# ShadenSmith/splatt

Measured on AMD Instinct MI355X. Metric: mttkrp_gflops, higher is better.
Workload: dtype f64; 1 GPU; model=amazon-shaped CPD-ALS, nnz=1741809018, cp_rank=16, csf=all, tiling=none, parallelism=medium-grid [1, 1, 1] x1 (RCCL/xGMI)

## Files before the change

### csrc/hip/launchers.hpp

```cpp
#pragma once
#include <cstdint>

namespace splatt_store {
struct bf16 { uint16_t v; };
}

namespace splatt {
namespace hip {

using splatt_store::bf16;

int kernels_arch();
const char * error_string(int rc);

template <typename V>
int mttkrp_csf3(int which, const int64_t * fptr0, const int32_t * fids0,
                const int64_t * fptr1, const int32_t * fids1,
                const int32_t * fids2, const V * vals, int64_t nslices,
                int64_t nfibs, int64_t nnz, const V * Ma, const V * Mb,
                V * out, int rank, void * stream);

template <typename V, typename S = V, typename VS = V>
int mttkrp_flat(const int32_t * key, const int64_t * rowptr, int64_t nrows,
                int64_t p0, const int32_t * const * idx,
                const S * const * mats, const VS * vals, int64_t nnz, V * out,
                int rank, int nother, void * stream);

template <typename V>
int mttkrp_flat5(const int32_t * key, const int32_t * const * idx,
                 const V * const * mats, const V * vals,
                 const int64_t * blk_start, const int64_t * blk_end,
                 const int32_t * blk_row0, int64_t nblocks, int32_t chunk,
                 int32_t dim0, V * out, int rank, int nother, void * stream);
template <typename V, typename S = V>
int mttkrp_flat6(const int32_t * pack, const S * const * mats,
                 const V * vals, const int64_t * blk_start,
                 const int64_t * blk_end, const int32_t * blk_row0,
                 int64_t nblocks, int32_t chunk, int32_t dim0, V * out,
                 int rank, int nother, void * stream);

template <typename VS>
int mttkrp_strip(const int32_t * key, const int32_t * const * idx,
                 const double * const * mats, const VS * vals,
                 const int32_t * s_row0, const int32_t * s_nrows,
                 const int32_t * s_flags, const int64_t * s_bounds,
                 int ngroups, int64_t nstrips, int tile_rows, int wgs,
                 int64_t nnz, double * out, int rank, int nother,
                 void * stream, uint32_t * pace, int pace_us);
int strip_wgs(int rank, int nother, bool vals32, int tile_rows);
int strip_wall_khz();

template <typename V>
int mttkrp_det6(const int32_t * pack, const V * const * mats, const V * vals,
                const int64_t * blk_start, const int64_t * blk_end,
                const int32_t * blk_row0, const int64_t * blk_bucket_p0,
                int64_t nblocks, int32_t chunk, int32_t dim0,
                int64_t nrows_out, int64_t nbuckets, V * outb, V * side,
                V * out, int rank, int nother, void * stream);
int64_t flat_det_ws(int64_t nnz, int rank);
template <typename V>
int mttkrp_flat_det(const int32_t * key, const int32_t * const * idx,
                    const V * const * mats, const V * vals, int64_t nnz,
                    V * out, V * side, int64_t side_elems, int rank,
                    int nother, void * stream);

template <typename V>
int gram(const V * A, int64_t n, int F, V * G, void * stream);
template <typename V>
int gram_det(const V * A, int64_t n, int F, V * Gpart, int64_t nparts, V * G,
             void * stream);
template <typename V>
int rowsolve(const V * A, const V * B, V * C, int64_t n, int F,
             void * stream);
template <typename V>
int spd_inverse(const V * G, V * Ginv, int F, void * stream);
int colacc(const double * A, int64_t n, int F, int which, double * out,
           void * stream);
int colscale(double * A, int64_t n, int F, const double * lam, void * stream);
int coldot(const double * X, const double * A, int64_t n, int F, double * out,
           void * stream);
int als_prep(const double * const * grams, int ngrams, double reg,
             double * Ginv, int F, double * zero_gram, double * lam_init,
             double * zero_inner, void * stream);

int als_tail(const double * K, const double * Ginv, int64_t n, int F,
             double * A, double * lam, double * gram, double * inner,
             void * stream);
int64_t als_tail_cap_rows();

int64_t complete_slot_elems(int F);
int complete_segments(const int32_t * const * idx,
                      const double * const * mats, int nother,
                      const double * vals, const int64_t * seg_start,
                      const int32_t * seg_len, const int32_t * seg_row,
                      const int32_t * seg_slot, int64_t seg0, int64_t nseg,
                      int64_t slot0, int F, double reg, double * ws,
                      double * out, void * stream);
int complete_reduce(const double * ws, const int32_t * mrow,
                    const int64_t * mslot, int64_t m0, int64_t nm,
                    int64_t slot0, int F, double reg, double * out,
                    void * stream);
// ... 35 lines not shown
```

### csrc/hip/mttkrp_strip.hip

```cpp
#include <hip/hip_runtime.h>
#include <cstdint>

#include <type_traits>

#include "device_common.hpp"
#include "launchers.hpp"

namespace {

constexpr int STRIP_THREADS = 1024;
constexpr int STRIP_PAD = 2;

template <typename T, int N>
__device__ __forceinline__ void ldnt_vec(const T * p, T (&r)[N]) {
  if constexpr (N == 1) {
    r[0] = ldnt(p);
  } else {
    using VT = T __attribute__((ext_vector_type(N)));
    const VT v = __builtin_nontemporal_load(reinterpret_cast<const VT *>(p));
    #pragma unroll
    for (int i = 0; i < N; ++i) r[i] = v[i];
  }
}

struct StripArgs {
  const int32_t * key, * i0, * i1, * i2;
  const double * m0, * m1, * m2;
  const int32_t * row0, * nrows, * flags;
  const int64_t * bounds;
  int ngroups;
  int64_t nnz;
  uint32_t * pace;
  int64_t budget;
};

constexpr int PACE_ARRIVALS = 0;
constexpr int PACE_TIMEOUTS = 32;
constexpr int PACE_LONGEST = 64;
constexpr int PACE_WORDS = 96;

template <int F, int NOTHER, typename VS>
__global__ void __launch_bounds__(STRIP_THREADS)
mttkrp_strip_kern(const StripArgs a, const VS * __restrict__ vals,
                  int64_t nstrips, int tile_rows,
                  double * __restrict__ out) {
  constexpr int R = WAVE / F;
  constexpr int W = 32;
  constexpr int EPL = (F >= W) ? 1 : W / F;
  constexpr int VPL = (sizeof(VS) == 8 && EPL > 1) ? EPL / 2 : EPL;
  constexpr int NVL = EPL / VPL;
  constexpr int CH = W / NVL;
  constexpr int GB = 8;
  constexpr int LD = F + STRIP_PAD;
  extern __shared__ double tile[];

  const int32_t * __restrict__ key = a.key;
  const int32_t * __restrict__ i0 = a.i0;
  const int32_t * __restrict__ i1 = a.i1;
  const int32_t * __restrict__ i2 = a.i2;
  const double * __restrict__ m0 = a.m0;
  const double * __restrict__ m1 = a.m1;
  const double * __restrict__ m2 = a.m2;

  uint32_t ticket = 0;
  bool waiting = true;
  int64_t longest = 0;
  auto pace = [&]() {
    if (!a.pace) return;
    __syncthreads();
    if (threadIdx.x == 0) {
      uint32_t * arrivals = a.pace + PACE_ARRIVALS;
      __hip_atomic_fetch_add(arrivals, 1u, __ATOMIC_RELAXED,
                             __HIP_MEMORY_SCOPE_AGENT);
      const uint32_t target = ++ticket * gridDim.x;
      if (waiting) {
        const int64_t t0 = (int64_t)wall_clock64();
        while (__hip_atomic_load(arrivals, __ATOMIC_RELAXED,
                                 __HIP_MEMORY_SCOPE_AGENT) < target) {
          if ((int64_t)wall_clock64() - t0 >= a.budget) {
            atomicAdd(a.pace + PACE_TIMEOUTS, 1u);
            waiting = false;
            break;
          }
          __builtin_amdgcn_s_sleep(8);
        }
        const int64_t dt = (int64_t)wall_clock64() - t0;
        if (dt > longest) longest = dt;
      }
    }
    __syncthreads();
  };

  const int lane = threadIdx.x & (WAVE - 1);
  const int c = lane % F;
  const int g = lane / F;
  const int gbase = g * F;
  const int slot = c & (W / EPL - 1);
  const int nlg = (blockDim.x / WAVE) * R;
  const int gid = (threadIdx.x / WAVE) * R + g;

  for (int64_t s = blockIdx.x; s - blockIdx.x < nstrips; s += gridDim.x) {
    if (s >= nstrips) {
      for (int grp = 0; grp < a.ngroups; ++grp) pace();
      break;
    }
    const int32_t row0 = a.row0[s];
    const int nr = a.nrows[s] < tile_rows ? a.nrows[s] : tile_rows;
    const int fl = a.flags[s];
    const int64_t * bnd = a.bounds + s * (a.ngroups + 1);

    for (int e = threadIdx.x; e < nr * LD; e += blockDim.x) tile[e] = 0.0;
    __syncthreads();

    int32_t cur = -1;
    double acc = 0.0;
    auto flush = [&]() {
      const uint32_t lr = (uint32_t)(cur - row0);
      if (lr < (uint32_t)nr) unsafeAtomicAdd(&tile[lr * LD + c], acc);
    };
    auto fold = [&](int32_t k, double x) {
      if (k != cur) {
        flush();
        acc = 0.0;
        cur = k;
      }
      acc += x;
    };
    auto scalar = [&](int64_t pa, int64_t pb) {
      for (int64_t p = pa; p < pb; ++p) {
        double x = (double)ldnt(&vals[p]) * m0[(int64_t)ldnt(&i0[p]) * F + c]
                   * ldnt(&m1[(int64_t)ldnt(&i1[p]) * F + c]);
        if constexpr (NOTHER > 2)
          x *= ldnt(&m2[(int64_t)ldnt(&i2[p]) * F + c]);
        fold(ldnt(&key[p]), x);
      }
    };

    for (int grp = 0; grp < a.ngroups; ++grp) {
      const int64_t p0 = bnd[grp], p1 = bnd[grp + 1];
      const int64_t wlo = p0 / W;
// ... 14 lines not shown
        #pragma unroll
        for (int k = 0; k < NVL; ++k)
          ldnt_vec(vals + pw + k * CH + slot * VPL, vreg[k]);
        #pragma unroll
        for (int k = 0; k < NVL; ++k) {
          #pragma unroll 1
          for (int h = 0; h < CH; h += GB) {
            const int ub = k * CH + h;
            double vv[GB], a0[GB], a1[GB], a2[GB];
            #pragma unroll
            for (int u = 0; u < GB; ++u) {
              const int src = gbase + ub / EPL + u / EPL;
              vv[u] = (double)__shfl(vreg[k][u % VPL],
                                     gbase + h / VPL + u / VPL, WAVE);
              const int32_t j0 = __shfl(i0reg[u % EPL], src, WAVE);
              const int32_t j1 = __shfl(i1reg[u % EPL], src, WAVE);
              a0[u] = m0[(int64_t)j0 * F + c];
              a1[u] = ldnt(&m1[(int64_t)j1 * F + c]);
              if constexpr (NOTHER > 2) {
                const int32_t j2 = __shfl(i2reg[u % EPL], src, WAVE);
                a2[u] = ldnt(&m2[(int64_t)j2 * F + c]);
              }
            }
            #pragma unroll
            for (int u = 0; u < GB; ++u) {
              double x = vv[u] * a0[u] * a1[u];
              if constexpr (NOTHER > 2) x *= a2[u];
              const int32_t k = __shfl(kreg[u % EPL],
                                       gbase + ub / EPL + u / EPL, WAVE);
              if (ub + u >= lo && ub + u < hi) fold(k, x);
            }
          }
        }
      }

      if (wend > whi && gid == nlg - 1)
        scalar(whi * W > p0 ? whi * W : p0, p1);
      if (grp + 1 < a.ngroups) pace();
    }
    flush();
    __syncthreads();

    for (int e = threadIdx.x; e < nr * F; e += blockDim.x) {
      const int lr = e / F, cc = e % F;
      const double v = tile[lr * LD + cc];
      double * o = &out[(int64_t)(row0 + lr) * F + cc];
      if ((lr == 0 && (fl & 1)) || (lr == nr - 1 && (fl & 2)))
        atomic_add_g(o, v);
      else
        *o = v;
    }
    if (a.pace) pace(); else __syncthreads();
  }
  if (a.pace && threadIdx.x == 0 && longest > 0)
    atomicMax(a.pace + PACE_LONGEST,
              (uint32_t)(longest < 0xFFFFFFFFll ? longest : 0xFFFFFFFFll));
}

inline int lds_limit() {
  static int limit = -1;
  if (limit < 0) {
    int dev = 0, v = 0;
    if (hipGetDevice(&dev) != hipSuccess
        || hipDeviceGetAttribute(&v, hipDeviceAttributeMaxSharedMemoryPerBlock,
                                 dev) != hipSuccess)
      return 0;
    limit = v;
  }
  return limit;
}

inline int cu_count() {
  static int n = -1;
  if (n < 0) {
    int dev = 0, v = 0;
    if (hipGetDevice(&dev) != hipSuccess
        || hipDeviceGetAttribute(&v, hipDeviceAttributeMultiprocessorCount,
                                 dev) != hipSuccess)
      return 0;
    n = v;
  }
  return n;
}

inline int wall_khz() {
  static int khz = -1;
  if (khz < 0) {
    int dev = 0, v = 0;
    if (hipGetDevice(&dev) != hipSuccess
        || hipDeviceGetAttribute(&v, hipDeviceAttributeWallClockRate, dev)
               != hipSuccess || v <= 0)
      return 0;
    khz = v;
  }
  return khz;
}

struct StripLaunch {
  StripArgs a;
  const void * vals;
  int64_t nstrips;
  int wgs;
  int tile_rows;
  double * out;
  hipStream_t st;
};

template <int F, int NOTHER, typename VS>
int strip_inst(const StripLaunch * L, int lds, int * wgs) {
  static int lds_set = 0;
  auto kern = mttkrp_strip_kern<F, NOTHER, VS>;
  if (lds > lds_set) {
    const hipError_t e = hipFuncSetAttribute(
        reinterpret_cast<const void *>(kern),
        hipFuncAttributeMaxDynamicSharedMemorySize, lds);
    if (e != hipSuccess) return (int)e;
    lds_set = lds;
  }
  if (!L) {
    int per_cu = 0;
    const hipError_t e = hipOccupancyMaxActiveBlocksPerMultiprocessor(
        &per_cu, kern, STRIP_THREADS, (size_t)lds);
    if (e != hipSuccess) return (int)e;
    *wgs = per_cu * cu_count();
    return wall_khz() > 0 ? 0 : (int)hipErrorInvalidDevice;
  }
  if (L->a.pace) {
    const hipError_t e = hipMemsetAsync(
        L->a.pace, 0, PACE_WORDS * sizeof(uint32_t), L->st);
    if (e != hipSuccess) return (int)e;
  }
  const int64_t n = L->nstrips < L->wgs ? L->nstrips : L->wgs;
  hipLaunchKernelGGL(kern, dim3((uint32_t)n), dim3(STRIP_THREADS),
                     (size_t)lds, L->st, L->a,
                     static_cast<const VS *>(L->vals), L->nstrips,
                     L->tile_rows, L->out);
  return launch_rc();
}

template <typename VS>
int strip_dispatch(const StripLaunch * L, int tile_rows, int rank, int nother,
                   int * wgs) {
  if (!(rank == 16 || rank == 32 || rank == 64) || nother < 2 || nother > 3
      || tile_rows < 1)
    return -1;
  const int64_t lds = (int64_t)tile_rows * (rank + STRIP_PAD) * 8;
  if (lds > lds_limit()) return -2;
#define SI(F_, N_) return strip_inst<F_, N_, VS>(L, (int)lds, wgs)
#define SF(N_) \
  switch (rank) { case 16: SI(16, N_); case 32: SI(32, N_); \
                  default: SI(64, N_); }
  if (nother == 2) { SF(2); }
  SF(3);
#undef SF
#undef SI
}

}

namespace splatt {
namespace hip {

int strip_wgs(int rank, int nother, bool vals32, int tile_rows) {
  int wgs = 0;
  const int rc = vals32
      ? strip_dispatch<float>(nullptr, tile_rows, rank, nother, &wgs)
      : strip_dispatch<double>(nullptr, tile_rows, rank, nother, &wgs);
  return rc == 0 ? wgs : 0;
}

template <typename VS>
int mttkrp_strip(const int32_t * key, const int32_t * const * idx,
                 const double * const * mats, const VS * vals,
                 const int32_t * s_row0, const int32_t * s_nrows,
                 const int32_t * s_flags, const int64_t * s_bounds,
                 int ngroups, int64_t nstrips, int tile_rows, int wgs,
                 int64_t nnz, double * out, int rank, int nother,
                 void * stream, uint32_t * pace, int pace_us) {
  if (nstrips <= 0) return 0;
  if (wgs < 1 || ngroups < 1 || nother < 2 || nother > 3 || pace_us < 0)
    return -1;
  uintptr_t bits = (uintptr_t)key | (uintptr_t)vals;
  for (int t = 0; t < nother; ++t) bits |= (uintptr_t)idx[t];
  if (bits & 127) return -1;
  StripLaunch L{{key, idx[0], idx[1], nother > 2 ? idx[2] : nullptr, mats[0],
                 mats[1], nother > 2 ? mats[2] : nullptr, s_row0, s_nrows,
                 s_flags, s_bounds, ngroups, nnz, pace,
                 (int64_t)pace_us * wall_khz() / 1000},
                vals, nstrips, wgs, tile_rows, out, (hipStream_t)stream};
  return strip_dispatch<VS>(&L, tile_rows, rank, nother, nullptr);
}

#define STRIP_SIG(VS)                                                      \
  const int32_t *, const int32_t * const *, const double * const *,        \
  const VS *, const int32_t *, const int32_t *, const int32_t *,           \
  const int64_t *, int, int64_t, int, int, int64_t, double *, int, int,    \
  void *, uint32_t *, int
template int mttkrp_strip<double>(STRIP_SIG(double));
template int mttkrp_strip<float>(STRIP_SIG(float));
#undef STRIP_SIG

int strip_wall_khz() { return wall_khz(); }

}
}
```

### csrc/pybind.cpp

```cpp
#include <torch/extension.h>
#include <array>
#include <string>
#include <vector>

#include "core/types.hpp"
#include "core/sptensor.hpp"
#include "core/csf.hpp"
#include "core/mttkrp_cpu.hpp"
#include "core/matrix.hpp"
#include "core/cpd.hpp"
#include "core/io.hpp"
#include "core/partition.hpp"
#include "hip/launchers.hpp"

namespace sp = splatt;
namespace gpu = splatt::hip;
using torch::Tensor;


template <typename T> struct Tag { using type = T; };
#define TAG_TYPE(tag) typename decltype(tag)::type

template <typename T>
static constexpr torch::ScalarType dtype_of() {
// ... 454 lines not shown
    rp = rowptr_ptr(*rowptr, out);
  }
  return gpu::mttkrp_flat<V, S, VS>(kp, rp, rp ? rowptr->numel() - 1 : 0, p0,
                                    ip.data(), mp.data(), vp, nnz, op, rank,
                                    (int)nother, (void *)stream);
}

static void py_gpu_mttkrp_flat(Tensor key, std::vector<Tensor> idx,
                               std::vector<Tensor> mats, Tensor vals,
                               Tensor out, int64_t stream) {
  TORCH_CHECK(!mats.empty(), "flat kernel supports 3..8 modes");
  by_store(vals, mats[0], [&](auto v, auto s) {
    using V = TAG_TYPE(v);
    using S = TAG_TYPE(s);
    const int rc = flat_launch<V, S, V>(c10::nullopt, 0, key, idx, mats, vals,
                                        out, stream);
    check_rc(rc, "flat MTTKRP",
             std::string(std::is_same<S, float>::value ? "f32" : "bf16")
             + " factor store needs rank in {4,8,16,32,64}");
  });
}

static bool py_gpu_mttkrp_flat_rp(Tensor rowptr, int64_t p0,
                                  std::vector<Tensor> idx,
                                  std::vector<Tensor> mats, Tensor vals,
                                  Tensor out, int64_t stream) {
  TORCH_CHECK(!mats.empty(), "flat kernel supports 3..8 modes");
  return by_store(vals, mats[0], [&](auto v, auto s) {
    using V = TAG_TYPE(v);
    const int rc = flat_launch<V, TAG_TYPE(s), V>(rowptr, p0, c10::nullopt,
                                                  idx, mats, vals, out,
                                                  stream);
    if (rc > 0) check_rc(rc, "flat MTTKRP");
    return rc == 0;
  });
}

static bool py_gpu_mttkrp_flat_v32(c10::optional<Tensor> rowptr, int64_t p0,
                                   c10::optional<Tensor> key,
                                   std::vector<Tensor> idx,
                                   std::vector<Tensor> mats, Tensor vals32,
                                   Tensor out, int64_t stream) {
  const int rc = flat_launch<double, double, float>(rowptr, p0, key, idx, mats,
                                                    vals32, out, stream);
  if (rc > 0) check_rc(rc, "flat MTTKRP");
  return rc == 0;
}

static bool py_mttkrp_strip_gpu(Tensor key, std::vector<Tensor> idx,
                                std::vector<Tensor> mats, Tensor vals,
                                Tensor s_row0, Tensor s_nrows, Tensor s_flags,
                                Tensor s_bounds, int64_t tile_rows,
                                int64_t wgs, Tensor out, int64_t stream,
                                c10::optional<Tensor> pace, int64_t pace_us) {
  const size_t nother = idx.size();
  TORCH_CHECK(nother >= 2 && nother <= 3, "strip kernel supports 3..4 modes");
  TORCH_CHECK(tile_rows >= 1 && tile_rows <= (1 << 20) && wgs >= 1
              && wgs <= (1 << 20), "tile_rows / wgs out of range");
  const int64_t nnz = vals.numel();
  const int rank = rank_of(mats);
  double * op = out_ptr<double>(out, rank);
  auto ip = stream_table(idx, nother, nnz);
  auto mp = factor_table<double>(mats, nother, rank);
  const int32_t * kp = dev_ptr<int32_t>(key, "key");
  TORCH_CHECK(key.numel() == nnz, "key must be int32 of nnz entries");
  const int32_t * r0 = dev_ptr<int32_t>(s_row0, "strip row0");
  const int32_t * nr = dev_ptr<int32_t>(s_nrows, "strip nrows");
  const int32_t * fl = dev_ptr<int32_t>(s_flags, "strip flags");
  const int64_t * bp = dev_ptr<int64_t>(s_bounds, "strip bounds");
  const int64_t ns = s_row0.numel();
  TORCH_CHECK(s_nrows.numel() == ns && s_flags.numel() == ns
              && s_bounds.dim() == 2 && s_bounds.size(0) == ns
              && s_bounds.size(1) >= 2 && s_bounds.size(1) <= (1 << 16),
              "strip descriptor lengths differ");
  const int ng = (int)s_bounds.size(1) - 1;
  uint32_t * pp = nullptr;
  if (pace.has_value()) {
    const Tensor & p = *pace;
    TORCH_CHECK(p.is_cuda(), "pace must be a device tensor");
    TORCH_CHECK(p.scalar_type() == torch::kInt32
                || p.scalar_type() == at::ScalarType::UInt32,
                "pace has dtype ", p.scalar_type(), ", expected Int or UInt32");
    TORCH_CHECK(p.is_contiguous() && p.numel() >= 96,
                "pace must be contiguous and hold at least 96 words");
    pp = static_cast<uint32_t *>(p.data_ptr());
  }
  TORCH_CHECK(pace_us >= 0 && pace_us <= 60 * 1000 * 1000,
              "pace_us out of range");
  const int rc = vals.scalar_type() == torch::kFloat32
      ? gpu::mttkrp_strip<float>(kp, ip.data(), mp.data(),
                                 dev_ptr<float>(vals, "vals"), r0, nr, fl, bp,
                                 ng, ns, (int)tile_rows, (int)wgs, nnz, op,
                                 rank, (int)nother, (void *)stream, pp,
                                 (int)pace_us)
      : gpu::mttkrp_strip<double>(kp, ip.data(), mp.data(),
                                  dev_ptr<double>(vals, "vals"), r0, nr, fl,
                                  bp, ng, ns, (int)tile_rows, (int)wgs, nnz,
                                  op, rank, (int)nother, (void *)stream, pp,
                                  (int)pace_us);
  if (rc > 0) check_rc(rc, "strip MTTKRP");
  return rc == 0;
}

static py::dict py_plan_strips(Tensor rowptr, int64_t tile_rows,
                               int64_t nnz_cap) {
  TORCH_CHECK(!rowptr.is_cuda() && rowptr.scalar_type() == torch::kInt64
              && rowptr.is_contiguous() && rowptr.numel() >= 1,
              "rowptr must be a contiguous host int64 tensor");
  TORCH_CHECK(tile_rows >= 1 && nnz_cap >= 1, "tile_rows, nnz_cap >= 1");
  const sp::Strips s = sp::plan_strips(rowptr.data_ptr<int64_t>(),
                                       rowptr.numel() - 1, tile_rows, nnz_cap);
  auto t32 = [](const std::vector<int32_t> & v) {
    return torch::tensor(v, torch::kInt32);
  };
  auto t64 = [](const std::vector<int64_t> & v) {
    return torch::tensor(v, torch::kInt64);
  };
  py::dict d;
  d["row0"] = t32(s.row0);
  d["nrows"] = t32(s.nrows);
  d["flags"] = t32(s.flags);
  d["p0"] = t64(s.p0);
  d["p1"] = t64(s.p1);
  return d;
}

static void py_gpu_mttkrp_flat_det(Tensor key, std::vector<Tensor> idx,
                                   std::vector<Tensor> mats, Tensor vals,
                                   Tensor out, Tensor side, int64_t stream) {
  const size_t nother = idx.size();
  TORCH_CHECK(nother >= 2 && nother <= 4,
              "deterministic kernel supports 3..5 modes");
  by_dtype(vals, [&](auto tag) {
    using V = TAG_TYPE(tag);
    const V * vp = dev_ptr<V>(vals, "vals");
    const int64_t nnz = vals.numel();
    const int rank = rank_of(mats);
    const int32_t * kp = dev_ptr<int32_t>(key, "key");
    TORCH_CHECK(key.numel() == nnz, "key must be int32 of nnz entries");
    auto ip = stream_table(idx, nother, nnz);
    auto mp = factor_table<V>(mats, nother, rank);
    const int rc = gpu::mttkrp_flat_det<V>(
        kp, ip.data(), mp.data(), vp, nnz, out_ptr<V>(out, rank),
        dev_ptr<V>(side, "side"), side.numel(), rank, (int)nother,
        (void *)stream);
    if (rc == -2)
      check_rc(rc, "deterministic MTTKRP", c10::str(
          "deterministic workspace too small (", side.numel(), " elems < ",
          gpu::flat_det_ws(nnz, rank), ")"));
    check_rc(rc, "deterministic MTTKRP", "deterministic kernel requires rank "
             "in {4,8,16,32,64} and <= 5 modes");
  });
// ... 444 lines not shown
                         gram.data_ptr<double>(), inner_ptr(inner, F),
                         (void *)stream),
           "als_tail",
           "als_tail kernel launch failed: rank or alignment does not qualify");
}

PYBIND11_MODULE(TORCH_EXTENSION_NAME, m) {
  m.def("gpu_als_prep", &py_gpu_als_prep,
        "Hadamard of Grams + SPD inverse + reset of the tail accumulators");
  m.def("gpu_als_tail", &py_gpu_als_tail,
        "fused ALS tail: A = (K Ginv)/lam, lam, gram += A^T A, inner");
  m.def("als_tail_cap_rows", &gpu::als_tail_cap_rows,
        "row count at which the fused tail's grid reaches its cap");
  m.def("gpu_admm_update", &py_gpu_admm_update,
        "fused block-ADMM factor update (in place on H, U)");
  m.def("hip_apr_update", &py_hip_apr_update,
        "CP-APR multiplicative row update of a root-sorted stream (f64)");
  m.def("gpu_ttmc", &py_gpu_ttmc,
        "TTMc of a root-sorted stream: one batch of segments + row folds");
  m.def("ttmc_max_cols", &gpu::ttmc_max_cols,
        "widest TTMc output row the HIP kernel supports");
  m.def("gpu_complete_update", &py_gpu_complete_update,
        "row-wise completion update: one batch of segments + row solves");
  m.def("complete_slot_elems", &gpu::complete_slot_elems,
        "workspace doubles per segment slot at a rank");
  m.def("gpu_kruskal_predict", &py_gpu_kruskal_predict,
        "Kruskal model values at COO coordinates");
  m.def("tensor_load", &py_tensor_load, "load .tns/.bin tensor");
  m.def("tns_write", &py_tns_write);
  m.def("bin_write", &py_bin_write);
  m.def("coo_fix", &py_coo_fix, "sort+dedup and/or remove empty slices");
  m.def("csf_build", &py_csf_build, "CPU CSF build for a level permutation");
  m.def("mttkrp_stream", &py_mttkrp_stream, "COO gold-oracle MTTKRP (CPU)");
  m.def("mttkrp_csf_cpu", &py_mttkrp_csf, "CSF MTTKRP (CPU)");
  m.def("cpd_als_cpu", &py_cpd_als, "CPD-ALS on the CPU reference path");
  m.def("seeded_init", &py_seeded_init, "partition-invariant seeded factor init");
  m.def("order_modes", &py_order_modes, "CSF mode-order policies");
  m.def("gpu_mttkrp3", &py_gpu_mttkrp3, "3-mode CSF MTTKRP HIP kernels");
  m.def("gpu_mttkrp_flat", &py_gpu_mttkrp_flat,
        "flat expanded-CSF MTTKRP HIP kernel (3..5 modes)");
  m.def("gpu_mttkrp_flat_rp", &py_gpu_mttkrp_flat_rp,
        "flat MTTKRP with row pointers in place of the key stream (root "
        "output, key-sorted stream); false = declined, use gpu_mttkrp_flat");
  m.def("gpu_mttkrp_flat_v32", &py_gpu_mttkrp_flat_v32,
        "flat MTTKRP (v7) reading an f32 copy of f32-exact f64 values, by "
        "row pointers or key stream; false = declined, use the f64 stream");
  m.def("mttkrp_strip_gpu", &py_mttkrp_strip_gpu,
        "strip/window flat MTTKRP (root output in LDS tiles over a "
        "strip-layout stream); false = declined, use gpu_mttkrp_flat",
        py::arg("key"), py::arg("idx"), py::arg("mats"), py::arg("vals"),
        py::arg("s_row0"), py::arg("s_nrows"), py::arg("s_flags"),
        py::arg("s_bounds"), py::arg("tile_rows"), py::arg("wgs"),
        py::arg("out"), py::arg("stream"), py::arg("pace") = py::none(),
        py::arg("pace_us") = 3600);
  m.def("strip_wall_khz", &gpu::strip_wall_khz,
        "rate of the wall clock of the strip kernel's pace words, kHz");
  m.def("strip_wgs", &gpu::strip_wgs,
        "resident workgroups of a strip kernel instance on this device "
        "(rank, nother, f32 values, tile rows); 0 = no such instance");
  m.def("plan_strips", &py_plan_strips,
        "strips of a root-sorted stream: row0/nrows/flags/p0/p1 (host)");
  m.def("gpu_mttkrp_flat_det", &py_gpu_mttkrp_flat_det,
        "bitwise-deterministic flat MTTKRP (depth-0 streams, spec ranks)");
  m.def("flat_det_ws_elems", &gpu::flat_det_ws,
        "workspace elements required by gpu_mttkrp_flat_det");
  m.def("gpu_gram", &py_gpu_gram, "G += A^T A (tall-skinny, F<=64)");
  m.def("gpu_colacc", &py_gpu_colacc,
        "out[f] (pre-zeroed) += sum_i A[i,f]^2 (which=0), or "
        "out[f] = max(out[f], max_i |A[i,f]|) (which=1)");
  m.def("gpu_colscale", &py_gpu_colscale, "A[i,f] /= lam[f] in place");
  m.def("gpu_coldot", &py_gpu_coldot,
        "out[f] (pre-zeroed) += sum_i X[i,f] * A[i,f]");
  m.def("gpu_gram_det", &py_gpu_gram_det,
        "G = A^T A, per-block partials folded in fixed order "
        "(bitwise-deterministic)");
  m.def("gpu_rowsolve", &py_gpu_rowsolve,
        "C = A @ B (B is FxF, staged in LDS; bitwise-deterministic)");
  m.def("gpu_spd_inverse", &py_gpu_spd_inverse,
        "Ginv = G^-1 for SPD FxF (F<=64), one-workgroup Cholesky");
  m.def("gpu_mttkrp_flat5", &py_gpu_mttkrp_flat5,
        "LDS-staged flat MTTKRP (bucketed builds, root output)");
  m.def("gpu_mttkrp_flat6", &py_gpu_mttkrp_flat6,
        "LDS-staged flat MTTKRP over the packed int4 stream");
  m.def("gpu_mttkrp_det6", &py_gpu_mttkrp_det6,
        "LDS-staged deterministic MTTKRP (bucket-privatized outputs)");
  m.def("partition_weighted", [](std::vector<int64_t> w, int nparts) {
    int64_t bn = 0;
    auto parts = sp::partition_weighted(w.data(), (int64_t)w.size(), nparts, &bn);
    return py::make_tuple(parts, bn);
  }, "optimal chains-on-chains partition (boundaries, bottleneck)");
  m.def("hip_arch", &gpu::kernels_arch);
}
```

### splatt_amd/__init__.py

```python

__version__ = "0.1.0"
VERSION = (0, 1, 0)

from splatt_amd.sptensor import SpTensor
from splatt_amd.csf import Csf, CsfSet, CsfAllocPolicy, build_csf, csf_alloc, order_modes
from splatt_amd.mttkrp import mttkrp, mttkrp_stream, strip_pace_stats
from splatt_amd.cpd import CpdOptions, Kruskal, cpd_als, cpd_als_cpu_native, seeded_init
from splatt_amd.kruskal import (kruskal_fit, kruskal_innerprod, kruskal_norm,
                                kruskal_to_dense)
from splatt_amd.completion import (CompleteOptions, Completion, complete_als,
                                   complete_update, kruskal_predict, rmse)
from splatt_amd.admm import (AoAdmmOptions, Constraint, ConstrainedKruskal,
                             admm_solve, admm_update, box, cpd_aoadmm, l1,
                             nonneg, nonneg_l1)
from splatt_amd.tucker import Tucker, TuckerOptions, ttmc, tucker_hooi
from splatt_amd.apr import AprOptions, PoissonKruskal, apr_update, cpd_apr

load = SpTensor.load

__all__ = [
    "SpTensor", "Csf", "CsfSet", "CsfAllocPolicy", "build_csf", "csf_alloc",
    "order_modes", "mttkrp", "mttkrp_stream", "strip_pace_stats",
    "CpdOptions", "Kruskal",
    "cpd_als", "cpd_als_cpu_native", "seeded_init", "load",
    "kruskal_fit", "kruskal_innerprod", "kruskal_norm", "kruskal_to_dense",
    "CompleteOptions", "Completion", "complete_als", "complete_update",
    "kruskal_predict", "rmse",
    "AoAdmmOptions", "Constraint", "ConstrainedKruskal", "admm_solve",
    "admm_update", "cpd_aoadmm", "nonneg", "l1", "nonneg_l1", "box",
    "Tucker", "TuckerOptions", "ttmc", "tucker_hooi",
    "AprOptions", "PoissonKruskal", "apr_update", "cpd_apr",
]
```

### splatt_amd/csf.py

```python
from __future__ import annotations

from dataclasses import dataclass
from enum import Enum
from typing import List, Optional, Sequence

import torch

from splatt_amd._ext import native
from splatt_amd.sptensor import SpTensor


class CsfAllocPolicy(str, Enum):
    ONEMODE = "one"
    TWOMODE = "two"
    ALLMODE = "all"


@dataclass
class Csf:
    dims: List[int]
    dim_perm: List[int]
    fptr: List[Optional[torch.Tensor]]
    fids: List[Optional[torch.Tensor]]
    vals: torch.Tensor
# ... 180 lines not shown
    groups = max(1, min(int(groups), nb))
    edge = torch.tensor([-(-g * nb // groups) for g in range(groups + 1)],
                        dtype=kdt, device=dev)
    q = (torch.arange(ns, dtype=kdt, device=dev) * nb).unsqueeze(1) + edge
    strips["bounds"] = torch.searchsorted(cell, q.reshape(-1).contiguous()) \
        .to(torch.int64).reshape(ns, groups + 1).cpu()
    return strips, order


def build_csf(t: SpTensor, perm: Sequence[int], flat_only: bool = False,
              gather_tiles: int = 0, stage_rank: int = 0,
              lds_kb: int = 0, strip_rows: int = 0, strip_cap: int = 0,
              strip_window: int = 0, strip_wgs: int = 0,
              strip_groups: int = 0) -> Csf:
    if any(d > 0xFFFFFFFF for d in t.dims):
        raise ValueError("mode dimensions above 2^32 are not supported "
                         "(CSF node ids are 32-bit; shard the mode first)")
    if t.device.type == "cuda":
        if any(d > 0x7FFFFFFF for d in t.dims):
            raise ValueError(
                "device builds support mode dimensions up to 2^31-1 "
                "(int32 stream labels; shard the mode or build on CPU)")
        if t.nnz > 0x7FFFFFFF:
            raise ValueError(
                "device builds support up to 2^31-1 nonzeros per shard "
                "(torch sort limit; shard the tensor or build on CPU)")
        if lds_kb <= 0:
            import os
            lds_kb = int(os.environ.get("SPLATT_LDS_KB", "24"))
        return _build_csf_device(t, list(perm), flat_only, gather_tiles,
                                 stage_rank, lds_kb,
                                 (strip_rows, strip_cap, strip_window,
                                  strip_wgs, strip_groups))
    d = native().csf_build(t.inds, t.vals, list(t.dims), list(perm))
    return Csf(dims=[int(x) for x in d["dims"]],
               dim_perm=[int(x) for x in d["dim_perm"]],
               fptr=[x if isinstance(x, torch.Tensor) else None for x in d["fptr"]],
               fids=[x if isinstance(x, torch.Tensor) else None for x in d["fids"]],
               vals=d["vals"])


def _strip_ok(t: SpTensor, stage_rank: int) -> bool:
    import os
    return (t.vals.dtype == torch.float64 and 3 <= t.nmodes <= 4
            and stage_rank in (16, 32, 64)
            and os.environ.get("SPLATT_DETERMINISTIC") != "1")


def _strip_wgs(rank: int, nother: int, tile_rows: int) -> int:
    return min(native().strip_wgs(rank, nother, v32, tile_rows)
               for v32 in (False, True))


STRIP_GROUP_KB = 16384


def _strip_groups(factor_bytes: int) -> int:
    import os
    kb = int(os.environ.get("SPLATT_STRIP_GROUP_KB", str(STRIP_GROUP_KB)))
    return max(1, -(-factor_bytes // (max(1, kb) * 1024)))


def _strip_default(t: SpTensor, perm: List[int], stage_rank: int):
    import os
    if os.environ.get("SPLATT_STRIP") == "0" or not _strip_ok(t, stage_rank):
        return None
    tile_kb = int(os.environ.get("SPLATT_STRIP_TILE_KB", "128"))
    window_kb = int(os.environ.get("SPLATT_STRIP_WINDOW_KB", "1024"))
    wgs = int(os.environ.get("SPLATT_STRIP_WGS", "0"))
    tile_rows = max(1, tile_kb * 1024 // (stage_rank * 8))
    held = _strip_wgs(stage_rank, t.nmodes - 1, tile_rows)
    if held <= 0:
        return None
    return strip_gate(t.dims, perm, t.nnz, stage_rank, wgs if wgs > 0 else held,
                      tile_kb, window_kb)


def _strip_forced(t: SpTensor, perm: List[int], stage_rank: int,
                  sizes: tuple) -> dict:
    rows, cap, window, wgs, groups = (int(x) for x in sizes)
    if not _strip_ok(t, stage_rank):
        raise ValueError(
            "the strip/window layout needs an f64 tensor of 3 or 4 modes, "
            "stage_rank in {16,32,64} and a non-deterministic build")
    w = max(range(1, t.nmodes), key=lambda l: t.dims[perm[l]])
    if window <= 0:
        window = max(1, (1 << 20) // (stage_rank * 8))
    if wgs <= 0:
        wgs = _strip_wgs(stage_rank, t.nmodes - 1, rows)
        if wgs <= 0:
            raise ValueError(f"a strip of {rows} rows at rank {stage_rank} "
                             "does not fit the device's LDS")
    return {"level": w, "tile_rows": rows, "window_rows": window,
            "wgs": wgs, "cap": cap, "groups": groups}


def _build_csf_device(t: SpTensor, perm: List[int],
                      flat_only: bool = False,
                      gather_tiles: int = 0, stage_rank: int = 0,
                      lds_kb: int = 48,
                      strip_sizes: tuple = (0, 0, 0, 0, 0)) -> Csf:
    stage_rank_in = stage_rank
    nm, nnz = t.nmodes, t.nnz
    dev = t.device
    if nnz == 0:
        c = Csf(dims=list(t.dims), dim_perm=list(perm),
                fptr=[torch.zeros(1, dtype=torch.int64, device=dev)
# ... 37 lines not shown
            min_run = int(_os.environ.get("SPLATT_STAGE_MIN_RUN", "8"))
            vbytes = {"f32": 4, "bf16": 2}.get(
                _os.environ.get("SPLATT_FACTOR_STORE", ""),
                t.vals.element_size())
            chunk_cap = max(64, (lds_kb * 1024) // (stage_rank * vbytes))
            root_dim = max(1, t.dims[perm[0]])
            min_bytes = int(_os.environ.get("SPLATT_STAGE_MIN_BYTES", "0"))
            big, chunk, tiles = -1, 0, 1
            for l in sorted(range(1, nm), key=lambda x: -t.dims[perm[x]]):
                d = t.dims[perm[l]]
                if d * stage_rank * vbytes < min_bytes:
                    continue
                ch = min(chunk_cap, d)
                ti = (d + ch - 1) // ch
                if ti <= 1 or nnz // (ti * root_dim) >= min_run:
                    big, chunk, tiles = l, ch, ti
                    break
            if big < 0:
                strip_cfg = _strip_default(t, perm, stage_rank)
                stage_rank = 0
        else:
            dim_big = t.dims[perm[big]]
            tiles = gather_tiles
            chunk = (dim_big + tiles - 1) // tiles
        if tiles > 1:
            bucket = torch.div(t.inds[perm[big]].index_select(0, order),
                               chunk, rounding_mode="floor")
            order = order.index_select(0, torch.argsort(bucket, stable=True))
        if stage_rank > 0:
            stage_meta = {"level": big, "chunk": int(chunk),
                          "nbuckets": int(tiles)}
    strip_meta = None
    if strip_cfg is not None:
        w = strip_cfg["level"]
        nrows = t.dims[perm[0]]
        ns_rows = -(-nrows // strip_cfg["tile_rows"])
        cap = strip_cfg.get("cap") or max(1, -(-nnz // ns_rows))
        strips, sorder = strip_layout(
            t.inds[perm[0]].index_select(0, order),
            t.inds[perm[w]].index_select(0, order), nrows, t.dims[perm[w]],
            strip_cfg["tile_rows"], cap, strip_cfg["window_rows"],
            strip_cfg.get("groups") or _strip_groups(
                t.dims[perm[w]] * stage_rank_in * 8))
        order = order.index_select(0, sorder)
        del sorder
        by_load = torch.argsort(strips["p1"] - strips["p0"], descending=True,
                                stable=True)
        strip_meta = dict(strip_cfg, cap=int(cap),
                          nbuckets=int(strips["nbuckets"]))
        strip_meta["groups"] = int(strips["bounds"].shape[1]) - 1
        for k in ("row0", "nrows", "flags", "p0", "p1", "bounds"):
            strip_meta[k] = strips[k].index_select(0, by_load).to(dev)
        strip_meta["pace"] = torch.zeros(96, dtype=torch.int32, device=dev)
    sinds = [t.inds[perm[l]].index_select(0, order) for l in range(nm)]
    svals = t.vals.index_select(0, order)

    if flat_only:
        c = Csf(dims=list(t.dims), dim_perm=list(perm),
                fptr=[None] * nm, fids=[None] * nm, vals=svals)
        import os as _os3
        if (stage_meta is not None and nm <= 4
                and _os3.environ.get("SPLATT_PACK") != "0"):
            lvl = stage_meta["level"]
            levels = [0, lvl] + [l for l in range(1, nm) if l != lvl]
            pack = torch.zeros(nnz, 4, dtype=torch.int32, device=dev)
            for col, l in enumerate(levels):
                pack[:, col] = sinds[l].to(torch.int32)
            cache = {l: pack[:, col] for col, l in enumerate(levels)}
            object.__setattr__(c, "_pack", pack)
            object.__setattr__(c, "_pack_levels", levels)
        else:
            cache = {l: sinds[l].to(torch.int32) for l in range(nm)}
        c.fids[nm - 1] = cache[nm - 1]
        object.__setattr__(c, "_expand_cache", cache)
        if stage_meta is not None:
            object.__setattr__(c, "_stage", stage_meta)
        if strip_meta is not None:
            object.__setattr__(c, "_strip", strip_meta)
        return c

    fptr: List[Optional[torch.Tensor]] = [None] * nm
    fids: List[Optional[torch.Tensor]] = [None] * nm
    change = torch.zeros(nnz, dtype=torch.bool, device=dev)
    change[0] = True
    starts_per_level: List[torch.Tensor] = []
    for l in range(nm - 1):
        if nnz > 1:
            change[1:] |= sinds[l][1:] != sinds[l][:-1]
        starts = change.nonzero(as_tuple=True)[0]
        starts_per_level.append(starts)
        fids[l] = sinds[l].index_select(0, starts).to(torch.int32)
    for l in range(nm - 1):
        starts = starts_per_level[l]
        if l < nm - 2:
            child = starts_per_level[l + 1]
            ptr = torch.searchsorted(child, starts)
            ptr = torch.cat([ptr, torch.tensor([child.numel()], device=dev)])
        else:
            ptr = torch.cat([starts, torch.tensor([nnz], device=dev)])
        fptr[l] = ptr.to(torch.int64)
    fids[nm - 1] = sinds[nm - 1].to(torch.int32)

    if fids[0] is not None and fids[0].numel() == t.dims[perm[0]]:
        fids[0] = None

    return Csf(dims=list(t.dims), dim_perm=list(perm),
# ... 54 lines not shown
```

### splatt_amd/mttkrp.py

```python
from __future__ import annotations

import os
from typing import List, Optional

import torch

from splatt_amd._ext import native
from splatt_amd.csf import Csf, CsfSet
from splatt_amd.sptensor import SpTensor


def mttkrp_stream(t: SpTensor, mats: List[torch.Tensor], mode: int) -> torch.Tensor:
    return native().mttkrp_stream(t.inds.cpu(), t.vals.cpu(), list(t.dims),
                                  [m.cpu() for m in mats], mode)


def _gpu_mttkrp_csf(c: Csf, depth: int, mats: List[torch.Tensor],
                    mode: int, out: torch.Tensor) -> None:
    nm = c.nmodes
    if nm != 3:
        raise NotImplementedError(
            f"the hierarchical walk kernels support 3-mode CSF, got {nm} "
            f"modes (use alg='flat')")
    if c.fptr[0] is None:
# ... 228 lines not shown

def _gpu_mttkrp_flat(c: Csf, depth: int, mats: List[torch.Tensor],
                     out: torch.Tensor, rows: tuple | None = None) -> None:
    nm = c.nmodes
    key = c.ancestor_expand(depth)
    rank = int(mats[0].shape[1])
    stream = torch.cuda.current_stream().cuda_stream
    storage = mats[0].dtype != c.vals.dtype
    packed = (getattr(c, "_pack", None) is not None
              and os.environ.get("SPLATT_NO_PACK") != "1")
    if _use_lds(c, depth, rank) and (packed or not storage):
        blocks = _stage_blocks(c, rows)
        lvl = blocks["level"]
        if int(blocks["start"].numel()) == 0:
            return
        pack = getattr(c, "_pack", None)
        if pack is not None and os.environ.get("SPLATT_NO_PACK") != "1":
            levels = c._pack_levels
            ms = [mats[c.dim_perm[l]].contiguous() for l in levels[1:]]
            native().gpu_mttkrp_flat6(
                pack, ms, c.vals, blocks["start"], blocks["end"],
                blocks["row0"], blocks["chunk"], c.dims[c.dim_perm[lvl]],
                out, stream)
            return
        idx = [c.ancestor_expand(lvl).contiguous()]
        ms = [mats[c.dim_perm[lvl]].contiguous()]
        for l in range(nm):
            if l in (depth, lvl):
                continue
            idx.append(c.ancestor_expand(l).contiguous())
            ms.append(mats[c.dim_perm[l]].contiguous())
        native().gpu_mttkrp_flat5(
            key.contiguous(), idx, ms, c.vals, blocks["start"],
            blocks["end"], blocks["row0"], blocks["chunk"],
            c.dims[c.dim_perm[lvl]], out, stream)
        return
    strip = getattr(c, "_strip", None) if depth == 0 else None
    if strip is not None:
        if rows is not None:
            raise ValueError("rows-restricted MTTKRP needs a key-sorted "
                             "stream for this mode")
        if rank in (16, 32, 64) and not storage and nm <= 4:
            lv = [strip["level"]] + [l for l in range(1, nm)
                                     if l != strip["level"]]
            idx = [c.ancestor_expand(l).contiguous() for l in lv]
            ms = [mats[c.dim_perm[l]].contiguous() for l in lv]
            v32 = _vals32(c, rank, mats)
            paced = os.environ.get("SPLATT_STRIP_PACE") != "0"
            if native().mttkrp_strip_gpu(
                    key.contiguous(), idx, ms, c.vals if v32 is None else v32,
                    strip["row0"], strip["nrows"], strip["flags"],
                    strip["bounds"], strip["tile_rows"],
                    strip["wgs"], out, stream,
                    strip["pace"] if paced else None, _strip_pace_us()):
                return
    p0, p1 = 0, c.nnz
    if rows is not None:
        if not _key_sorted(c, depth):
            raise ValueError("rows-restricted MTTKRP needs a key-sorted "
                             "stream for this mode")
        p0, p1 = _key_bounds(c, depth, rows[0], rows[1])
        if p0 >= p1:
            return
    idx, ms = [], []
    for l in range(nm):
        if l == depth:
            continue
        idx.append(c.ancestor_expand(l)[p0:p1].contiguous())
        ms.append(mats[c.dim_perm[l]].contiguous())
    v32 = _vals32(c, rank, mats)
    if v32 is not None:
        if flat_rowptr_ok(c, depth, rank):
            if native().gpu_mttkrp_flat_v32(_root_rowptr(c), p0, None, idx,
                                            ms, v32[p0:p1], out, stream):
                return
        elif native().gpu_mttkrp_flat_v32(None, 0, key[p0:p1].contiguous(),
                                          idx, ms, v32[p0:p1], out, stream):
            return
    if flat_rowptr_ok(c, depth, rank) and native().gpu_mttkrp_flat_rp(
            _root_rowptr(c), p0, idx, ms, c.vals[p0:p1], out, stream):
        return
    native().gpu_mttkrp_flat(key[p0:p1].contiguous(), idx, ms,
                             c.vals[p0:p1], out, stream)


def factor_store_dtype():
    env = os.environ.get("SPLATT_FACTOR_STORE", "")
    return {"f32": torch.float32, "bf16": torch.bfloat16}.get(env)


STRIP_PACE_US = 3600


def _strip_pace_us() -> int:
    return max(0, int(os.environ.get("SPLATT_STRIP_PACE_US",
                                     str(STRIP_PACE_US))))


def strip_pace_stats(c: Csf) -> tuple:
    words = c._strip["pace"].cpu().tolist()
    khz = native().strip_wall_khz()
    return (words[0] & 0xFFFFFFFF, words[32] & 0xFFFFFFFF,
            (words[64] & 0xFFFFFFFF) * 1000.0 / khz if khz > 0 else 0.0)


def mttkrp_rows_ok(src: CsfSet | Csf, mode: int, rank: int) -> bool:
    if isinstance(src, CsfSet):
        c = src.csfs[src.mode_csf[mode]]
        depth = src.mode_depth[mode]
    else:
        c, depth = src, src.level_of_mode(mode)
    if os.environ.get("SPLATT_DETERMINISTIC") == "1":
        return False
    if c.device.type == "cuda" and _use_lds(c, depth, rank):
        return True
    if depth == 0 and getattr(c, "_strip", None) is not None:
        return False
    return _key_sorted(c, depth)


def mttkrp(src: CsfSet | Csf, mats: List[torch.Tensor], mode: int,
           out: Optional[torch.Tensor] = None,
           nthreads: int = 0, alg: str = "flat",
           deterministic: Optional[bool] = None,
           rows: Optional[tuple] = None) -> torch.Tensor:
    if isinstance(src, CsfSet):
        c = src.csfs[src.mode_csf[mode]]
        depth = src.mode_depth[mode]
    else:
        c = src
        depth = c.level_of_mode(mode)

    if not 0 <= mode < c.nmodes:
        raise IndexError(f"mode {mode} out of range for {c.nmodes} modes")
    if len(mats) != c.nmodes:
        raise ValueError(f"need {c.nmodes} factor matrices, got {len(mats)}")
    rank = int(mats[0].shape[1])
    storage = (c.device.type == "cuda" and c.vals.dtype == torch.float64
               and mats[0].dtype in (torch.float32, torch.bfloat16))
    for m, A in enumerate(mats):
        if A.shape != (c.dims[m], rank):
            raise ValueError(
                f"factor {m} has shape {tuple(A.shape)}, expected "
                f"({c.dims[m]}, {rank})")
        if (A.dtype != c.vals.dtype and not storage) or A.device != c.device:
            raise ValueError(
                f"factor {m}: dtype/device {A.dtype}/{A.device} does not "
                f"match tensor {c.vals.dtype}/{c.device}")
    if storage and rank not in (4, 8, 16, 32, 64):
# ... 50 lines not shown
```

Before: 1506 GFLOP/s.

## Relax strip pacing barrier to slotted run-ahead and shrink strip groups

Replaces the single global arrival counter used to pace workgroups in the strip MTTKRP kernel with a ring of eight padded slot counters. Each workgroup may now run a configurable number of tickets ahead (default one) before waiting on older arrivals. This is meant to cut stall time at each pacing point while keeping workgroups roughly in step so factor rows stay cache-resident. The change also lowers the pacing timeout and halves the strip group size, and adds wait-time statistics and optional per-workgroup tracing. The run-ahead lets workgroups drift further apart, which risks more cache misses, and the stats add shared-memory updates and extra atomics.

```diff
diff --git a/csrc/hip/launchers.hpp b/csrc/hip/launchers.hpp
--- a/csrc/hip/launchers.hpp
+++ b/csrc/hip/launchers.hpp
@@ -46,7 +46,9 @@
                  const int32_t * s_flags, const int64_t * s_bounds,
                  int ngroups, int64_t nstrips, int tile_rows, int wgs,
                  int64_t nnz, double * out, int rank, int nother,
-                 void * stream, uint32_t * pace, int pace_us);
+                 void * stream, uint32_t * pace, int pace_us,
+                 uint32_t * slots = nullptr, int ahead = 0,
+                 uint32_t * trace = nullptr);
 int strip_wgs(int rank, int nother, bool vals32, int tile_rows);
 int strip_wall_khz();
 
diff --git a/csrc/hip/mttkrp_strip.hip b/csrc/hip/mttkrp_strip.hip
--- a/csrc/hip/mttkrp_strip.hip
+++ b/csrc/hip/mttkrp_strip.hip
@@ -32,12 +32,20 @@
   int64_t nnz;
   uint32_t * pace;
   int64_t budget;
+  uint32_t * slots;
+  int ahead;
+  uint32_t * trace;
 };
 
 constexpr int PACE_ARRIVALS = 0;
 constexpr int PACE_TIMEOUTS = 32;
 constexpr int PACE_LONGEST = 64;
+constexpr int PACE_WAITSUM = 65;
+constexpr int PACE_POLLED = 66;
 constexpr int PACE_WORDS = 96;
+constexpr int PACE_SLOTS = 8;
+constexpr int SLOT_STRIDE = 32;
+constexpr int SLOT_WORDS = PACE_SLOTS * SLOT_STRIDE;
 
 template <int F, int NOTHER, typename VS>
 __global__ void __launch_bounds__(STRIP_THREADS)
@@ -64,19 +72,35 @@
 
   uint32_t ticket = 0;
   bool waiting = true;
-  int64_t longest = 0;
+  __shared__ uint32_t pstat[3];
+  if (threadIdx.x == 0) pstat[0] = pstat[1] = pstat[2] = 0;
   auto pace = [&]() {
     if (!a.pace) return;
     __syncthreads();
     if (threadIdx.x == 0) {
-      uint32_t * arrivals = a.pace + PACE_ARRIVALS;
-      __hip_atomic_fetch_add(arrivals, 1u, __ATOMIC_RELAXED,
+      const uint32_t t = ticket++;
+      uint32_t * arrive = a.pace + PACE_ARRIVALS;
+      uint32_t * watch = arrive;
+      uint32_t target = ticket * gridDim.x;
+      bool wait = waiting;
+      if (a.slots) {
+        const uint32_t R = (uint32_t)a.ahead;
+        arrive = a.slots + (t % PACE_SLOTS) * SLOT_STRIDE;
+        wait = waiting && t >= R;
+        if (wait) {
+          const uint32_t u = t - R;
+          watch = a.slots + (u % PACE_SLOTS) * SLOT_STRIDE;
+          target = (u / PACE_SLOTS + 1) * gridDim.x;
+        }
+      }
+      __hip_atomic_fetch_add(arrive, 1u, __ATOMIC_RELAXED,
                              __HIP_MEMORY_SCOPE_AGENT);
-      const uint32_t target = ++ticket * gridDim.x;
-      if (waiting) {
+      if (wait) {
         const int64_t t0 = (int64_t)wall_clock64();
-        while (__hip_atomic_load(arrivals, __ATOMIC_RELAXED,
+        bool spun = false;
+        while (__hip_atomic_load(watch, __ATOMIC_RELAXED,
                                  __HIP_MEMORY_SCOPE_AGENT) < target) {
+          spun = true;
           if ((int64_t)wall_clock64() - t0 >= a.budget) {
             atomicAdd(a.pace + PACE_TIMEOUTS, 1u);
             waiting = false;
@@ -84,8 +108,14 @@
           }
           __builtin_amdgcn_s_sleep(8);
         }
-        const int64_t dt = (int64_t)wall_clock64() - t0;
-        if (dt > longest) longest = dt;
+        const int64_t dt64 = (int64_t)wall_clock64() - t0;
+        const uint32_t dt =
+            (uint32_t)(dt64 < 0xFFFFFFFFll ? dt64 : 0xFFFFFFFFll);
+        if (dt > pstat[0]) pstat[0] = dt;
+        if (spun) {
+          pstat[1] = pstat[1] + dt < dt ? 0xFFFFFFFFu : pstat[1] + dt;
+          ++pstat[2];
+        }
       }
     }
     __syncthreads();
@@ -206,9 +236,23 @@
     }
     if (a.pace) pace(); else __syncthreads();
   }
-  if (a.pace && threadIdx.x == 0 && longest > 0)
-    atomicMax(a.pace + PACE_LONGEST,
-              (uint32_t)(longest < 0xFFFFFFFFll ? longest : 0xFFFFFFFFll));
+  if (a.pace && threadIdx.x == 0) {
+    const uint32_t lw = pstat[0], ws = pstat[1], polled = pstat[2];
+    if (lw > 0) atomicMax(a.pace + PACE_LONGEST, lw);
+    if (polled > 0) {
+      atomicAdd(a.pace + PACE_WAITSUM, ws);
+      atomicAdd(a.pace + PACE_POLLED, polled);
+    }
+    if (a.slots) atomicAdd(a.pace + PACE_ARRIVALS, ticket);
+    if (a.trace) {
+      const uint32_t xcc = __builtin_amdgcn_s_getreg(20 | (3 << 11));
+      uint32_t * tr = a.trace + (size_t)blockIdx.x * 4;
+      tr[0] = xcc;
+      tr[1] = ws;
+      tr[2] = polled;
+      tr[3] = lw;
+    }
+  }
 }
 
 inline int lds_limit() {
@@ -282,6 +326,11 @@
   if (L->a.pace) {
     const hipError_t e = hipMemsetAsync(
         L->a.pace, 0, PACE_WORDS * sizeof(uint32_t), L->st);
+    if (e != hipSuccess) return (int)e;
+  }
+  if (L->a.slots) {
+    const hipError_t e = hipMemsetAsync(
+        L->a.slots, 0, SLOT_WORDS * sizeof(uint32_t), L->st);
     if (e != hipSuccess) return (int)e;
   }
   const int64_t n = L->nstrips < L->wgs ? L->nstrips : L->wgs;
@@ -330,9 +379,13 @@
                  const int32_t * s_flags, const int64_t * s_bounds,
                  int ngroups, int64_t nstrips, int tile_rows, int wgs,
                  int64_t nnz, double * out, int rank, int nother,
-                 void * stream, uint32_t * pace, int pace_us) {
+                 void * stream, uint32_t * pace, int pace_us,
+                 uint32_t * slots, int ahead, uint32_t * trace) {
   if (nstrips <= 0) return 0;
   if (wgs < 1 || ngroups < 1 || nother < 2 || nother > 3 || pace_us < 0)
+    return -1;
+  if (ahead < 0 || ahead >= PACE_SLOTS || (ahead > 0 && !slots)
+      || ((slots || trace) && !pace))
     return -1;
   uintptr_t bits = (uintptr_t)key | (uintptr_t)vals;
   for (int t = 0; t < nother; ++t) bits |= (uintptr_t)idx[t];
@@ -340,7 +393,7 @@
   StripLaunch L{{key, idx[0], idx[1], nother > 2 ? idx[2] : nullptr, mats[0],
                  mats[1], nother > 2 ? mats[2] : nullptr, s_row0, s_nrows,
                  s_flags, s_bounds, ngroups, nnz, pace,
-                 (int64_t)pace_us * wall_khz() / 1000},
+                 (int64_t)pace_us * wall_khz() / 1000, slots, ahead, trace},
                 vals, nstrips, wgs, tile_rows, out, (hipStream_t)stream};
   return strip_dispatch<VS>(&L, tile_rows, rank, nother, nullptr);
 }
@@ -349,7 +402,7 @@
   const int32_t *, const int32_t * const *, const double * const *,        \
   const VS *, const int32_t *, const int32_t *, const int32_t *,           \
   const int64_t *, int, int64_t, int, int, int64_t, double *, int, int,    \
-  void *, uint32_t *, int
+  void *, uint32_t *, int, uint32_t *, int, uint32_t *
 template int mttkrp_strip<double>(STRIP_SIG(double));
 template int mttkrp_strip<float>(STRIP_SIG(float));
 #undef STRIP_SIG
diff --git a/csrc/pybind.cpp b/csrc/pybind.cpp
--- a/csrc/pybind.cpp
+++ b/csrc/pybind.cpp
@@ -530,7 +530,9 @@
                                 Tensor s_row0, Tensor s_nrows, Tensor s_flags,
                                 Tensor s_bounds, int64_t tile_rows,
                                 int64_t wgs, Tensor out, int64_t stream,
-                                c10::optional<Tensor> pace, int64_t pace_us) {
+                                c10::optional<Tensor> pace, int64_t pace_us,
+                                c10::optional<Tensor> slots, int64_t ahead,
+                                c10::optional<Tensor> trace) {
   const size_t nother = idx.size();
   TORCH_CHECK(nother >= 2 && nother <= 3, "strip kernel supports 3..4 modes");
   TORCH_CHECK(tile_rows >= 1 && tile_rows <= (1 << 20) && wgs >= 1
@@ -565,17 +567,39 @@
   }
   TORCH_CHECK(pace_us >= 0 && pace_us <= 60 * 1000 * 1000,
               "pace_us out of range");
+  auto words = [](const Tensor & p, const char * what, int64_t need) {
+    TORCH_CHECK(p.is_cuda(), what, " must be a device tensor");
+    TORCH_CHECK(p.scalar_type() == torch::kInt32
+                || p.scalar_type() == at::ScalarType::UInt32,
+                what, " has dtype ", p.scalar_type(),
+                ", expected Int or UInt32");
+    TORCH_CHECK(p.is_contiguous() && p.numel() >= need, what,
+                " must be contiguous and hold at least ", need, " words");
+    return static_cast<uint32_t *>(p.data_ptr());
+  };
+  TORCH_CHECK(ahead >= 0 && ahead <= 7, "ahead out of range 0..7");
+  uint32_t * sp_ = nullptr, * tp = nullptr;
+  if (slots.has_value()) {
+    TORCH_CHECK(pp != nullptr, "slots need a pace tensor");
+    sp_ = words(*slots, "slots", 256);
+  }
+  TORCH_CHECK(ahead == 0 || sp_ != nullptr,
+              "ahead > 0 needs pace and slots tensors");
+  if (trace.has_value()) {
+    TORCH_CHECK(pp != nullptr, "trace needs a pace tensor");
+    tp = words(*trace, "trace", 4 * std::min<int64_t>(wgs, ns));
+  }
   const int rc = vals.scalar_type() == torch::kFloat32
       ? gpu::mttkrp_strip<float>(kp, ip.data(), mp.data(),
                                  dev_ptr<float>(vals, "vals"), r0, nr, fl, bp,
                                  ng, ns, (int)tile_rows, (int)wgs, nnz, op,
                                  rank, (int)nother, (void *)stream, pp,
-                                 (int)pace_us)
+                                 (int)pace_us, sp_, (int)ahead, tp)
       : gpu::mttkrp_strip<double>(kp, ip.data(), mp.data(),
                                   dev_ptr<double>(vals, "vals"), r0, nr, fl,
                                   bp, ng, ns, (int)tile_rows, (int)wgs, nnz,
                                   op, rank, (int)nother, (void *)stream, pp,
-                                  (int)pace_us);
+                                  (int)pace_us, sp_, (int)ahead, tp);
   if (rc > 0) check_rc(rc, "strip MTTKRP");
   return rc == 0;
 }
@@ -1126,7 +1150,8 @@
         py::arg("s_row0"), py::arg("s_nrows"), py::arg("s_flags"),
         py::arg("s_bounds"), py::arg("tile_rows"), py::arg("wgs"),
         py::arg("out"), py::arg("stream"), py::arg("pace") = py::none(),
-        py::arg("pace_us") = 3600);
+        py::arg("pace_us") = 2200, py::arg("slots") = py::none(),
+        py::arg("ahead") = 0, py::arg("trace") = py::none());
   m.def("strip_wall_khz", &gpu::strip_wall_khz,
         "rate of the wall clock of the strip kernel's pace words, kHz");
   m.def("strip_wgs", &gpu::strip_wgs,
diff --git a/splatt_amd/__init__.py b/splatt_amd/__init__.py
--- a/splatt_amd/__init__.py
+++ b/splatt_amd/__init__.py
@@ -4,7 +4,8 @@
 
 from splatt_amd.sptensor import SpTensor
 from splatt_amd.csf import Csf, CsfSet, CsfAllocPolicy, build_csf, csf_alloc, order_modes
-from splatt_amd.mttkrp import mttkrp, mttkrp_stream, strip_pace_stats
+from splatt_amd.mttkrp import (mttkrp, mttkrp_stream, strip_pace_stats,
+                               strip_pace_waits)
 from splatt_amd.cpd import CpdOptions, Kruskal, cpd_als, cpd_als_cpu_native, seeded_init
 from splatt_amd.kruskal import (kruskal_fit, kruskal_innerprod, kruskal_norm,
                                 kruskal_to_dense)
@@ -21,6 +22,7 @@
 __all__ = [
     "SpTensor", "Csf", "CsfSet", "CsfAllocPolicy", "build_csf", "csf_alloc",
     "order_modes", "mttkrp", "mttkrp_stream", "strip_pace_stats",
+    "strip_pace_waits",
     "CpdOptions", "Kruskal",
     "cpd_als", "cpd_als_cpu_native", "seeded_init", "load",
     "kruskal_fit", "kruskal_innerprod", "kruskal_norm", "kruskal_to_dense",
diff --git a/splatt_amd/csf.py b/splatt_amd/csf.py
--- a/splatt_amd/csf.py
+++ b/splatt_amd/csf.py
@@ -256,7 +256,7 @@
                for v32 in (False, True))
 
 
-STRIP_GROUP_KB = 16384
+STRIP_GROUP_KB = 8192
 
 
 def _strip_groups(factor_bytes: int) -> int:
@@ -400,6 +400,7 @@
         for k in ("row0", "nrows", "flags", "p0", "p1", "bounds"):
             strip_meta[k] = strips[k].index_select(0, by_load).to(dev)
         strip_meta["pace"] = torch.zeros(96, dtype=torch.int32, device=dev)
+        strip_meta["slots"] = torch.zeros(256, dtype=torch.int32, device=dev)
     sinds = [t.inds[perm[l]].index_select(0, order) for l in range(nm)]
     svals = t.vals.index_select(0, order)
 
diff --git a/splatt_amd/mttkrp.py b/splatt_amd/mttkrp.py
--- a/splatt_amd/mttkrp.py
+++ b/splatt_amd/mttkrp.py
@@ -304,7 +304,10 @@
                     strip["row0"], strip["nrows"], strip["flags"],
                     strip["bounds"], strip["tile_rows"],
                     strip["wgs"], out, stream,
-                    strip["pace"] if paced else None, _strip_pace_us()):
+                    strip["pace"] if paced else None, _strip_pace_us(),
+                    strip["slots"] if paced else None,
+                    _strip_ahead() if paced else 0,
+                    _strip_trace(strip) if paced else None):
                 return
     p0, p1 = 0, c.nnz
     if rows is not None:
@@ -341,12 +344,41 @@
     return {"f32": torch.float32, "bf16": torch.bfloat16}.get(env)
 
 
-STRIP_PACE_US = 3600
+STRIP_PACE_US = 2200
 
 
 def _strip_pace_us() -> int:
     return max(0, int(os.environ.get("SPLATT_STRIP_PACE_US",
                                      str(STRIP_PACE_US))))
+
+
+STRIP_AHEAD = 1
+
+
+def _strip_ahead() -> int:
+    r = int(os.environ.get("SPLATT_STRIP_AHEAD", str(STRIP_AHEAD)))
+    if not 0 <= r <= 7:
+        raise ValueError(f"SPLATT_STRIP_AHEAD must be in 0..7, got {r}")
+    return r
+
+
+def _strip_trace(strip: dict):
+    if os.environ.get("SPLATT_STRIP_TRACE") != "1":
+        return None
+    tr = strip.get("trace")
+    if tr is None and not torch.cuda.is_current_stream_capturing():
+        grid = min(int(strip["wgs"]), int(strip["row0"].numel()))
+        tr = torch.zeros(grid, 4, dtype=torch.int32,
+                         device=strip["pace"].device)
+        strip["trace"] = tr
+    return tr
+
+
+def strip_pace_waits(c: Csf) -> tuple:
+    words = c._strip["pace"].cpu().tolist()
+    khz = native().strip_wall_khz()
+    return ((words[65] & 0xFFFFFFFF) * 1000.0 / khz if khz > 0 else 0.0,
+            words[66] & 0xFFFFFFFF)
 
 
 def strip_pace_stats(c: Csf) -> tuple:
```

New measurement: 1566 GFLOP/s, median of 6. 1.04x the previous value.
